# ecmwf/anemoi-core

Measured on AMD Instinct MI355X. Metric: forward nodes*channels/sec on O96 GraphTransformer, higher is better.
Workload: dtype bf16; 1 GPU; AnemoiModelEncProcDec forward, O96 data grid (40320 nodes, 84 vars x 2 steps) -> icosphere res 5 hidden mesh (10242 nodes, 81840 edges), GraphTransformer processor 16 layers x 512 ch x 16 heads, enc 62912 / dec 120960 edges, batch 1; parallelism=single GPU, hip_graph=True, graph_equals_eager=True, graph_segments=1

## Files before the change

### anemoi_core_amd/_lib.py

```python
from __future__ import annotations

import ctypes as C
import os
import threading

ABI_VERSION = 18
LIB_PATH = os.path.join(os.path.dirname(os.path.abspath(__file__)), "lib", "libanemoi_hip.so")

F32, BF16, F16 = 0, 1, 2
ACT_NONE, ACT_GELU = 0, 1
E_INVALID, E_UNSUPPORTED, E_LAUNCH = -1, -2, -3

_p, _i64, _i32, _f = C.c_void_p, C.c_int64, C.c_int32, C.c_float



class LinearPlan(C.Structure):
    _fields_ = [(name, _i32) for name in ("kernel", "tile_m", "tile_n", "pingpong", "stage_k", "mi", "wr", "kg", "stages", "epi", "main_rows",
                                          "tail_rows", "ln_tail_begin")]


SIGNATURES = {
    "anemoi_hip_abi_version": ([], C.c_int),
    "anemoi_hip_last_error": ([], C.c_char_p),
    "anemoi_gt_attention_fwd": ([_p, _i64, _p, _i64, _p, _i64, _p, _i64, _p, _p, _p, _i64, _p, _i64, _p, _i32, _i32, _i32, _i32, C.c_int, _p], C.c_int),
    "anemoi_gt_attention_bwd": ([_p, _i64, _p, _i64, _p, _i64, _p, _i64, _p, _i64, _p, _p, _i64, _p, _p, _p, _p, _p,
                                 _p, _i64, _p, _i64, _p, _i64, _p, _i64, _p, _p, _i32, _i32, _i32, _i32, _i32, C.c_int, _p], C.c_int),
    "anemoi_gt_attention_dropout_fwd": ([_p, _i64, _p, _i64, _p, _i64, _p, _i64, _p, _p, _p, _i64, _p, _i64, _p, _i32, _i32, _i32, _i32, _f, C.c_uint64,
                                         C.c_int, _p], C.c_int),
    "anemoi_gt_attention_dropout_bwd": ([_p, _i64, _p, _i64, _p, _i64, _p, _i64, _p, _i64, _p, _p, _i64, _p, _p, _p, _p, _p,
                                         _p, _i64, _p, _i64, _p, _i64, _p, _i64, _p, _p, _i32, _i32, _i32, _i32, _i32, _f, C.c_uint64, C.c_int, _p], C.c_int),
    "anemoi_attention_dropout_mask": ([_p, _i32, _i32, _f, C.c_uint64, _p], C.c_int),
    "anemoi_gt_attention_fused_edge_fwd": ([_p, _i64, _p, _i64, _p, _i64, _p, _i32, _p, _p, _p, _p, _p, _i64, _p, _i64, _p, _i32, _i32, _i32, _i32, C.c_int, _p], C.c_int),
    "anemoi_pack_edge_weights": ([_p, _p, _p, _i32, _i32, _i32, C.c_int, _p], C.c_int),
    "anemoi_pack_edge_features": ([_p, _i64, _p, _i32, _i32, _i32, C.c_int, _p], C.c_int),
    "anemoi_reduce_workspace_bytes": ([_i32], _i64),
    "anemoi_layernorm_bwd": ([_p, _i64, _p, _p, _i64, _p, _i64, _p, _p, _p, _i32, _i32, _f, C.c_int, _p], C.c_int),
    "anemoi_colsum": ([_p, _i64, _p, _p, _i32, _i32, C.c_int, _p], C.c_int),
    "anemoi_gelu_fwd": ([_p, _i64, _p, _i64, _i32, _i32, C.c_int, _p], C.c_int),
# ... 7 lines not shown
    "anemoi_assemble_output_norm": ([_p, _i64, C.c_int, _p, _i64, _p, _p, _p, _p, _i64, _i32, _i32, C.c_int, _p], C.c_int),
    "anemoi_affine_columns": ([_p, _i64, _p, _i64, _p, _p, _i32, _i32, _i32, C.c_int, _p], C.c_int),
    "anemoi_bound_columns": ([_p, _i64, _i32, _i32, _p, _p, _i32, C.c_int, _p], C.c_int),
    "anemoi_layernorm_fwd": ([_p, _i64, _p, _p, _p, _i64, _p, _i64, _i32, _i32, _f, C.c_int, _p], C.c_int),
    "anemoi_gt_attention_fused_edge_bwd_partial_floats": ([_i32, _i32, _i32], _i64),
    "anemoi_gt_attention_fused_edge_bwd": ([_p, _i64, _p, _i64, _p, _i64, _p, _i32, _p, _p, _i64, _p, _p, _i64, _p, _p, _p, _p, _p,
                                            _p, _i64, _p, _i64, _p, _i64, _p, _p, _p, _p, _p, _p, _p, _p, _i64, _p, _i64,
                                            _i32, _i32, _i32, _i32, _i32, C.c_int, _p], C.c_int),
    "anemoi_linear_wgrad_workspace_bytes": ([_i32, _i32, _i32], _i64),
    "anemoi_linear_wgrad": ([_p, _i64, _p, _i64, _p, _i64, _p, _p, _i32, _i32, _i32, C.c_int, _p], C.c_int),
    "anemoi_linear_splitk_f32": ([_p, _i64, _p, _i64, _p, _i64, _i32, _i32, _i32, _i32, C.c_int, _p], C.c_int),
    "anemoi_linear_stats_fwd": ([_p, _i64, _i32, _p, _i64, _p, _p, _i64, _p, _i64, _p, _i32, _i32, C.c_int, _p], C.c_int),
    "anemoi_linear_lnfold_fwd": ([_p, _i64, _i32, _p, _i64, _p, _p, _p, _i32, _f, C.c_int, _p, _i64, _i32, _i32, C.c_int, _p], C.c_int),
    "anemoi_linear_plan": ([_i32, _i32, _i32, _i32, _i32, _i32, C.c_int, C.POINTER(LinearPlan)], C.c_int),
    "anemoi_linear_fwd": ([_p, _i64, _i32, _p, _i64, _i32, _p, _i64, _p, _p, _i64, _p, _p, _i64, _p, _p, _i64, _p, _i64, _i32, _i32, C.c_int, C.c_int, _p], C.c_int),
    "anemoi_linear_fwd_pre": ([_p, _i64, _i32, _p, _i64, _i32, _p, _i64, _p, _p, _i64, _p, _p, _i64, _p, _p, _i64, _p, _i64, _p, _i64, _i32, _i32,
                               C.c_int, C.c_int, _p], C.c_int),
    "anemoi_edge_ln_residual_segment_sum_fwd": ([_p, _i64, _p, _i64, _p, _p, _f, _p, _p, _i64, _p, _i64, _i32, _i32, C.c_int, _p], C.c_int),
    "anemoi_segment_sum_rows": ([_p, _i64, _p, _p, _p, _i64, _i32, _i32, C.c_int, _p], C.c_int),
    "anemoi_gather_add_rows": ([_p, _i64, _p, _i64, _p, _p, _i64, _i32, _i32, C.c_int, _p], C.c_int),
    "anemoi_transpose_pad": ([_p, _i64, _p, _i64, _i32, _i32, _i32, C.c_int, _p], C.c_int),
    "anemoi_glu_fwd": ([_p, _i64, _p, _i64, _i32, _i32, _i32, C.c_int, _p], C.c_int),
    "anemoi_glu_bwd": ([_p, _i64, _p, _i64, _p, _i64, _i32, _i32, _i32, C.c_int, _p], C.c_int),
    "anemoi_gather_rows": ([_p, _i64, _p, _p, _i64, _i32, _i32, C.c_int, _p], C.c_int),
    "anemoi_peer_alloc": ([C.POINTER(_p), _i64, _i32], C.c_int),
    "anemoi_peer_free": ([_p], C.c_int),
    "anemoi_peer_export": ([_p, _p], C.c_int),
    "anemoi_peer_open": ([_p, C.POINTER(_p)], C.c_int),
    "anemoi_peer_close": ([_p], C.c_int),
    "anemoi_gt_chain_rows_per_tile": ([_i32], C.c_int),
    "anemoi_gt_chain2_fwd": ([_p, C.c_int, _p], C.c_int),
    "anemoi_gt_rowchain_fwd": ([_p, C.c_int, _p], C.c_int),
    "anemoi_gt_rowchain_panels_fwd": ([_p, C.c_int32, C.c_int32, C.c_int, _p], C.c_int),
    "anemoi_gt_chain2_side_fwd": ([_p, _p, C.c_int32, C.c_int32, C.c_int32, C.c_int, _p], C.c_int),
    "anemoi_gt_cluster_chain_fwd": ([_p, C.c_int, _p], C.c_int),
    "anemoi_gt_cluster_chain_workspace_bytes": ([], _i64),
    "anemoi_gnn_edge_chain_fwd": ([_p, _i64, _p, _i64, _p, _p, _i64, _p, _p, _p, _p, _p, _p, _p, _p, _p, _f, _p, _i64, _i32, _i32, C.c_int, _p], C.c_int),
    "anemoi_gnn_mlp_chain_fwd": ([_p, _i64, _i32, _p, _p, _p, _p, _p, _p, _p, _p, _f, _p, _i64, _p, _i64, _i32, _i32, C.c_int, _p], C.c_int),
    "anemoi_gnn_node_chain_segsum_fwd": ([_p, _i64, _p, _i64, _p, _p, _p, _p, _p, _p, _p, _p, _p, _f, _p, _i64, _p, _p, _i32, _p, _i64, _i32, _i32,
                                          C.c_int, _p], C.c_int),
    "anemoi_gnn_node_chain_fwd": ([_p, _i64, _p, _i64, _p, _p, _p, _p, _p, _p, _p, _p, _f, _p, _i64, _p, _p, _i32, _p, _i64, _i32, _i32, C.c_int, _p], C.c_int),
    "anemoi_peer_exchange_rows": ([_p, _i64, _p, _p, _i32, _i32, _i32, _p, _p, _i64, _p], C.c_int),
    "anemoi_window_attention_fwd": ([_p, _i64, _p, _i64, _p, _i64, _p, _i64, _p, _i32, _i32, _i32, _i32, _i32, _f, _f, _p, C.c_int, _p], C.c_int),
    "anemoi_sparse_project_fwd": ([_p, _i64, _i64, _i32, _i64, _i32, _i32, _p, _p, _p, _p, _p, _p, _p, _i64, _i64, _i32, _i32, _i32, C.c_int, C.c_int, _p], C.c_int),
}


EXPERIMENT_SIGNATURES = {
    "anemoi_gt_chain_fwd": ([_p, C.c_int, _p], C.c_int),
    "anemoi_gnn_edge_chain_timeline": ([_p, _i64, _p, _i64, _p, _p, _i64, _p, _p, _p, _p, _p, _p, _p, _p, _p, _f, _p, _i64, _i32, _p, _p], C.c_int),
}


class HipLibraryError(RuntimeError):
    pass


_lock = threading.Lock()
_lib = None


def load(path: str | None = None):
    global _lib
    if _lib is not None:
        return _lib
    with _lock:
# ... 40 lines not shown
```

### anemoi_core_amd/build.py

```python
from __future__ import annotations

import os
import shutil
import subprocess
import sys
from concurrent.futures import ThreadPoolExecutor

PKG = os.path.dirname(os.path.abspath(__file__))
REPO = os.path.dirname(PKG)
CSRC = os.path.join(PKG, "csrc")
LIBDIR = os.path.join(PKG, "lib")
LIBPATH = os.path.join(LIBDIR, "libanemoi_hip.so")
EXT_PATH = os.path.join(LIBDIR, "libanemoi_torch.so")
INCLUDE = os.path.join(REPO, "include")

SOURCES = ["lib.cpp", "gt_attention.hip", "gt_attention_bwd.hip", "rowwise.hip", "rowwise_bwd.hip", "linear.hip", "wgrad.hip", "peer.hip", "gt_chain2.hip", "gt_chain2_side.hip", "gt_rowchain.hip", "gt_cluster_chain.hip", "gnn_chain.hip", "window_attention.hip", "sparse_project.hip"]
EXPERIMENT_SOURCES = ["experiments/gt_chain.hip", "experiments/gnn_chain2.hip"]
EXP_LIBPATH = os.path.join(LIBDIR, "libanemoi_hip_exp.so")
ARCH = "gfx950"


def _hipcc() -> str:
    for cand in (os.environ.get("HIPCC"), shutil.which("hipcc"), "/opt/rocm/bin/hipcc"):
        if cand and os.path.exists(cand):
            return cand
    raise RuntimeError("hipcc not found (need ROCm >= 7.0)")


def _newer(target: str, deps: list[str]) -> bool:
    if not os.path.exists(target):
        return False
    t = os.path.getmtime(target)
    return all(os.path.getmtime(d) <= t for d in deps)


def _deps(path: str, dirs: list[str], seen: set | None = None) -> list[str]:
    import re

    seen = set() if seen is None else seen
    if path in seen:
        return []
    seen.add(path)
    out = [path]
    for inc in re.findall(r'^\s*#include\s+"([^"]+)"', open(path).read(), flags=re.M):
        for d in [os.path.dirname(path), *dirs]:
            cand = os.path.join(d, inc)
            if os.path.exists(cand):
                out += _deps(cand, dirs, seen)
                break
# ... 65 lines not shown
```

### anemoi_core_amd/layers/mapper.py

```python
from __future__ import annotations

import os
from typing import Optional

import torch
from torch import Tensor, nn

from .. import ops
from ..distributed import primitives as comm
from ..distributed.partition import (
    build_graph_partition_from_shard_info,
    ensure_edges_are_dst_sorted,
    local_bipartite_graph,
    shard_edges_1hop,
)
from ..distributed.shapes import BipartiteGraphShardInfo, comm_rank, comm_size, get_shard_sizes, model_is_distributed
from .block import GraphConvMapperBlock, GraphTransformerMapperBlock
from .handoff import Carrier, SideJob, inference_in, plain_layer_norm
from .kernels import PaddedLinear
from .mlp import MLP
from .utils import compute_mlp_hidden_dim, load_layer_kernels
from ..utils.tensors import version


_ROW_CHAIN = os.environ.get("ANEMOI_ROW_CHAIN", "1") != "0"
_ROW_CHAIN_MIN_ROWS = int(os.environ.get("ANEMOI_ROW_CHAIN_MIN_ROWS", "4096"))
_TAIL_PROJ = os.environ.get("ANEMOI_TAIL_PROJ", "1") != "0"
_ENC_DST_CACHE = os.environ.get("ANEMOI_ENC_DST_CACHE", "1") != "0"
_ROW_CHAIN_GEMM_BAND = tuple(int(v) for v in os.environ.get("ANEMOI_ROW_CHAIN_GEMM_BAND", "16384:262144").split(":"))


class _LocalGraphCache:

    def __init__(self, keep: int = 4):
        self.entries: dict = {}
        self.keep = keep

    def get(self, key, build):
        hit = self.entries.get(key)
        if hit is None:
            hit = build()
            if len(self.entries) >= self.keep:
                self.entries.pop(next(iter(self.entries)))
            self.entries[key] = hit
        return hit


class BaseMapper(nn.Module):
    def __init__(self, *, in_channels_src: int, in_channels_dst: int, hidden_dim: int, out_channels_dst: Optional[int] = None,
                 cpu_offload: bool = False, gradient_checkpointing: bool = True, layer_kernels=None, **kwargs) -> None:
        super().__init__()
        self.in_channels_src = in_channels_src
        self.in_channels_dst = in_channels_dst
        self.hidden_dim = hidden_dim
        self.out_channels_dst = out_channels_dst
        self.gradient_checkpointing = gradient_checkpointing
        self.layer_factory = load_layer_kernels(layer_kernels)
        if cpu_offload:
            raise NotImplementedError("cpu_offload is a training memory feature; not needed with 288 GB of HBM")
        self._local = _LocalGraphCache()
        self._heads_cache = None

# ... 52 lines not shown

    def _tail_projection(self):
        return None

    def _row_chain_ok(self, x: Tensor, lin, ln, projs: list, band: bool = True) -> bool:
        return (_ROW_CHAIN and x.is_cuda and x.dim() == 2 and x.dtype != torch.float32 and x.shape[0] >= _ROW_CHAIN_MIN_ROWS
                and not (band and _ROW_CHAIN_GEMM_BAND[0] < x.shape[0] < _ROW_CHAIN_GEMM_BAND[1])
                and self.hidden_dim == ops.CHAIN_CHANNELS and plain_layer_norm(ln) and lin.in_features <= x.shape[1] and lin.bias is not None
                and ops.gt_row_chain_supported(x, sum(p.out_features for p in projs)) and all(p.in_features == ops.CHAIN_CHANNELS for p in projs)
                and inference_in(x, lin, ln, *projs))

    def _row_chain_operands(self, x: Tensor, lin, side: str, band: bool = True):
        blk = self.proc
        ln = blk.layer_norm_attention_src if side == "src" else blk.layer_norm_attention_dest
        projs = [blk.lin_key, blk.lin_value] if side == "src" else [blk.lin_query, blk.lin_self]
        if not self._row_chain_ok(x, lin, ln, projs, band):
            return None
        params = [lin.weight, lin.bias, ln.weight, ln.bias] + [q for m in projs for q in (m.weight, m.bias)]
        K = x.shape[1]

        def build():
            w = lin.weight if lin.in_features == K else torch.nn.functional.pad(lin.weight, (0, K - lin.in_features))
            wq = torch.cat([m.weight for m in projs], dim=0)
            bq = torch.cat([m.bias if m.bias is not None else m.weight.new_zeros(m.out_features) for m in projs])
            wqg, dq = ops.fold_layer_norm(wq, bq, ln.weight, ln.bias)
            return ops.pack_embedding_frag(w), ops.pack_weight_frag(wqg), torch.cat([lin.bias.float(), dq]).to(x.dtype).contiguous(), wq.shape[0]

        return (*blk._fused.derived(f"rowchain:{side}:{K}", params, build), ln.eps)

    def _row_chain(self, x: Tensor, lin, side: str, want_x: bool):
        operands = self._row_chain_operands(x, lin, side)
        return None if operands is None else ops.gt_row_chain(x, *operands, want_x_out=want_x)

    def _static_row_chain(self, x: Tensor, lin):
        blk = self.proc
        ln, projs = blk.layer_norm_attention_dest, [blk.lin_query, blk.lin_self]
        params = [x, lin.weight, lin.bias, ln.weight, ln.bias] + [q for m in projs for q in (m.weight, m.bias)]
        return blk._fused.derived(f"rowchain-static:dst:{x.shape[1]}", params, lambda: (self._row_chain(x, lin, "dst", True), x))[0]

    def destination_side_job(self, x_dst: Tensor, panels_per_rider: int) -> Optional[SideJob]:
        operands = self._row_chain_operands(x_dst, self.emb_nodes_dst, "dst", band=False)
        if operands is None:
            return None
        we, wqg, vec, q_out, eps = operands
        n, dt, dev = x_dst.shape[0], x_dst.dtype, x_dst.device
        return SideJob(x=x_dst, we=we, wqg=wqg, vec=vec, q_out_features=q_out, ln_eps=eps, y=torch.empty((n, self.hidden_dim), dtype=dt, device=dev),
                       q=torch.empty((n, q_out), dtype=dt, device=dev), panels_per_rider=panels_per_rider)

    def _embed(self, padded: PaddedLinear, x: Tensor, lin, side: str, carrier: Optional[Carrier]) -> Tensor:
        ln = self.proc.layer_norm_attention_src if side == "src" else self.proc.layer_norm_attention_dest
        if carrier is not None and side == "dst" and carrier.side_job is not None and carrier.side_job.x is x:
            job, carrier.side_job = carrier.side_job, None
            job.finish()
            return carrier.put(job.y, proj=job.q)
        if carrier is not None:
            if _ENC_DST_CACHE and side == "dst" and carrier.static_dst is x and not torch.is_grad_enabled():
                r = self._static_row_chain(x, lin)
            else:
                r = self._row_chain(x, lin, side, want_x=side == "dst" or self.proc.update_src_nodes)
            if r is not None:
                y, proj = r
                return carrier.put(y if y is not None else x.new_empty((x.shape[0], 0)), proj=proj)
            if self.proc._ln_fold_ok(ln, x):
                y, stats = padded.with_row_stats(x, lin)
                return y if stats is None else carrier.put(y, stats=stats)
        return padded(x, lin)

    @comm.scoped_forward
    def forward(self, x, batch_size: int, shard_info: BipartiteGraphShardInfo, edge_attr: Tensor, edge_index: Tensor,
                model_comm_group=None, keep_x_dst_sharded: bool = False, edges_are_dst_sorted: bool = True, cond=None, **kwargs):
        if self.shard_strategy == "heads" and model_is_distributed(model_comm_group):
            return self._forward_heads(x, batch_size, shard_info, edge_attr, edge_index, model_comm_group, keep_x_dst_sharded,
                                       edges_are_dst_sorted, cond=cond, **kwargs)
        x_src, x_dst = x
        edge_attr, edge_index = ensure_edges_are_dst_sorted(
            edge_attr, edge_index, edges_are_sharded=shard_info.edges_are_sharded(), model_comm_group=model_comm_group,
            edges_are_dst_sorted=edges_are_dst_sorted)
        g = self._local_graph(x, shard_info, edge_attr, edge_index, model_comm_group)
        d0, d1 = g["dst_range"]
        sharded = model_is_distributed(model_comm_group)
        if sharded and not shard_info.dst_is_sharded():
            x_dst = x_dst[d0:d1]
        if sharded and shard_info.src_is_sharded():
            x_src_c, g["plans"]["src"] = comm.exchange_rows(x_src, g["src_ids"], shard_info.src_nodes, model_comm_group,
                                                            gather_fn=ops.gather_rows, plan=g["plans"].get("src"))
        elif g["all_connected"]:
            x_src_c = x_src
        else:
# ... 204 lines not shown
```

### anemoi_core_amd/ops.py

```python
from __future__ import annotations

from dataclasses import dataclass
from typing import NamedTuple, Optional

import os

import torch
from torch import Tensor

from . import _ext, _lib

_DT = {torch.float32: _lib.F32, torch.bfloat16: _lib.BF16, torch.float16: _lib.F16}


def _dt(t: Tensor) -> int:
    try:
        return _DT[t.dtype]
    except KeyError:
        raise ValueError(f"unsupported dtype {t.dtype}; supported: float32, bfloat16, float16") from None


try:
    _raw_stream = torch._C._cuda_getCurrentRawStream
except AttributeError:
# ... 1069 lines not shown
    q_out = torch.empty((N, q_out_features), dtype=dt, device=x.device)
    a = _row_chain_args(x, we, wqg, vec, q_out_features, ln_eps, x_out, q_out, rows_per_tile)
    _lib.check(_lib.load().anemoi_gt_rowchain_fwd(_lib.C.byref(a), _dt(x), _stream()), "gt_rowchain_fwd")
    return x_out, q_out


def gt_row_chain_panels(x: Tensor, we: Tensor, wqg: Tensor, vec: Tensor, q_out_features: int, ln_eps: float, y: Optional[Tensor], q: Tensor,
                        first_panel: int, panels: int) -> None:
    a = _row_chain_args(x, we, wqg, vec, q_out_features, ln_eps, y, q, 0)
    _lib.check(_lib.load().anemoi_gt_rowchain_panels_fwd(_lib.C.byref(a), int(first_panel), int(panels), _dt(x), _stream()), "gt_rowchain_panels_fwd")


def _row_chain_args(x: Tensor, we: Tensor, wqg: Tensor, vec: Tensor, q_out_features: int, ln_eps: float, x_out: Optional[Tensor], q_out: Tensor,
                    rows_per_tile: int) -> _RowChainArgs:
    _dev(x, we, wqg, vec, x_out, q_out)
    N, K = x.shape
    dt, D = x.dtype, CHAIN_CHANNELS
    if not gt_row_chain_supported(x, q_out_features):
        raise NotImplementedError(f"gt_row_chain: x {tuple(x.shape)} {dt} / q_out={q_out_features} (16-bit rows of <= {D} columns, a multiple of 8; q_out a multiple of {D})")
    kp = (K + 127) // 128 * 128
    for name, w, numel in (("we", we, D * kp), ("wqg", wqg, q_out_features * D)):
        if w.dim() != 1 or w.numel() != numel or w.dtype != dt or not w.is_contiguous():
            raise ValueError(f"gt_row_chain: {name} must be the contiguous fragment-major image ({numel} x {dt})")
    if vec.dim() != 1 or vec.numel() != D + q_out_features or vec.dtype != dt or not vec.is_contiguous():
        raise ValueError(f"gt_row_chain: vec must be contiguous [{D + q_out_features}] {dt} = cat[be, dq]")
    for name, t, cols in (("x_out", x_out, D), ("q_out", q_out, q_out_features)):
        if t is not None and (tuple(t.shape) != (N, cols) or t.dtype != dt or not t.is_contiguous()):
            raise ValueError(f"gt_row_chain: {name} must be contiguous [{N}, {cols}] {dt}")
    xp, ldx = _rows(x, "x", dt)
    return _RowChainArgs(xp, ldx, K, we.data_ptr(), wqg.data_ptr(), q_out_features, vec.data_ptr(), float(ln_eps),
                         0 if x_out is None else x_out.data_ptr(), D, q_out.data_ptr(), q_out_features, N, D, int(rows_per_tile))


def gnn_edge_chain(e: Tensor, g1: Tensor, idx1: Tensor, g2: Tensor, idx2: Tensor, w0: Tensor, b0: Tensor, w1: Tensor, b1: Tensor, w2: Tensor,
                   b2: Tensor, ln_w: Tensor, ln_b: Optional[Tensor], eps: float) -> Tensor:
    _dev(e, g1, idx1, g2, idx2, w0, b0, w1, b1, w2, b2, ln_w, ln_b)
    M, D = e.shape
    dt = e.dtype
    if D != CHAIN_CHANNELS or dt not in (torch.bfloat16, torch.float16):
        raise NotImplementedError(f"gnn_edge_chain: {D} channels / {dt} (built for {CHAIN_CHANNELS} channels, 16-bit dtypes)")
    for name, w in (("w0", w0), ("w1", w1), ("w2", w2)):
        if w.dim() != 1 or w.numel() != D * D or w.dtype != dt or not w.is_contiguous():
            raise ValueError(f"gnn_edge_chain: {name} must be the fragment-major image of a [{D}, {D}] weight (pack_weight_frag)")
    for name, ix in (("idx1", idx1), ("idx2", idx2)):
        if ix.dtype != torch.int32 or ix.dim() != 1 or ix.shape[0] != M or not ix.is_contiguous():
            raise ValueError(f"gnn_edge_chain: {name} must be contiguous int32 [{M}]")
    if g1.shape[1] != D or g2.shape[1] != D:
        raise ValueError("gnn_edge_chain: the gathered tables must have 512 columns")
    out = torch.empty((M, D), dtype=dt, device=e.device)
    (ep, lde), (p1, ld1), (p2, ld2) = _rows(e, "e", dt), _rows(g1, "g1", dt), _rows(g2, "g2", dt)
    _lib.check(_lib.load().anemoi_gnn_edge_chain_fwd(ep, lde, p1, ld1, idx1.data_ptr(), p2, ld2, idx2.data_ptr(), w0.data_ptr(), _vec(b0, "b0", D, dt),
                                                     w1.data_ptr(), _vec(b1, "b1", D, dt), w2.data_ptr(), _vec(b2, "b2", D, dt), _vec(ln_w, "ln_w", D, dt),
                                                     _vec(ln_b, "ln_b", D, dt), float(eps), out.data_ptr(), D, M, D, _dt(e), _stream()), "gnn_edge_chain_fwd")
    return out


def gnn_mlp_chain(x: Tensor, w0: Tensor, b0: Tensor, w1: Tensor, b1: Tensor, w2: Tensor, b2: Tensor, ln_w: Tensor, ln_b: Optional[Tensor],
                  eps: float, residual: Optional[Tensor] = None) -> Tensor:
    _dev(x, w0, b0, w1, b1, w2, b2, ln_w, ln_b, residual)
    N, K = x.shape
    D, dt = CHAIN_CHANNELS, x.dtype
    if dt not in (torch.bfloat16, torch.float16) or K % 128 or not 128 <= K <= D:
        raise NotImplementedError(f"gnn_mlp_chain: width {K} / {dt} (built for 16-bit rows of 128, 256, 384 or 512 columns)")
    for name, w, numel in (("w0", w0, D * K), ("w1", w1, D * D), ("w2", w2, D * D)):
        if w.dim() != 1 or w.numel() != numel or w.dtype != dt or not w.is_contiguous():
            raise ValueError(f"gnn_mlp_chain: {name} must be a contiguous fragment-major image of {numel} elements (pack_weight_frag)")
# ... 231 lines not shown
```

### include/anemoi_hip.h

```cpp
#ifndef ANEMOI_HIP_H
#define ANEMOI_HIP_H

#include <stdint.h>

#ifdef __cplusplus
extern "C" {
#endif

#define ANEMOI_HIP_ABI_VERSION 18

typedef enum { ANEMOI_F32 = 0, ANEMOI_BF16 = 1, ANEMOI_F16 = 2 } anemoi_dtype_t;
typedef enum { ANEMOI_ACT_NONE = 0, ANEMOI_ACT_GELU = 1 } anemoi_act_t;

#define ANEMOI_OK 0
#define ANEMOI_E_INVALID (-1)
#define ANEMOI_E_UNSUPPORTED (-2)
#define ANEMOI_E_LAUNCH (-3)

int anemoi_hip_abi_version(void);
const char* anemoi_hip_last_error(void);

int anemoi_gt_attention_fwd(const void* q, int64_t ldq, const void* k, int64_t ldk, const void* v, int64_t ldv,
                            const void* e, int64_t lde, const int32_t* row, const int32_t* colptr,
                            const void* addend, int64_t ldadd, void* out, int64_t ldo, float* lse,
                            int32_t n_dst, int32_t n_src, int32_t H, int32_t C, anemoi_dtype_t dtype, void* stream);

int anemoi_gt_attention_bwd(const void* q, int64_t ldq, const void* k, int64_t ldk, const void* v, int64_t ldv,
                            const void* e, int64_t lde, const void* out, int64_t ldo, const float* lse,
                            const void* d_out, int64_t lddo, const int32_t* row, const int32_t* colptr,
                            const int32_t* rowptr, const int32_t* edge_ids, const int32_t* edge_dst,
                            void* dq, int64_t lddq, void* dk, int64_t lddk, void* dv, int64_t lddv, void* de, int64_t ldde,
                            float* p_ws, float* ds_ws, int32_t n_dst, int32_t n_src, int32_t n_edges, int32_t H, int32_t C,
                            anemoi_dtype_t dtype, void* stream);

int anemoi_gt_attention_dropout_fwd(const void* q, int64_t ldq, const void* k, int64_t ldk, const void* v, int64_t ldv,
                                    const void* e, int64_t lde, const int32_t* row, const int32_t* colptr,
                                    const void* addend, int64_t ldadd, void* out, int64_t ldo, float* lse,
                                    int32_t n_dst, int32_t n_src, int32_t H, int32_t C, float drop_p, uint64_t drop_seed,
                                    anemoi_dtype_t dtype, void* stream);
int anemoi_gt_attention_dropout_bwd(const void* q, int64_t ldq, const void* k, int64_t ldk, const void* v, int64_t ldv,
                                    const void* e, int64_t lde, const void* out, int64_t ldo, const float* lse,
                                    const void* d_out, int64_t lddo, const int32_t* row, const int32_t* colptr,
// ... 141 lines not shown
                              int64_t timeout_ticks, void* stream);

typedef struct anemoi_gt_chain2_args {
  const void* attn;   int64_t ld_attn;
  const void* x_res;  int64_t ld_x;
  const void* wp;
  const void* w1;     int32_t hidden;
  const void* w2;
  const void* wq;     int32_t q_out_features;
  const void* vec;
  float ln1_eps;      float lnq_eps;
  const void* extra;  int64_t ld_extra;
  void* x_out;        int64_t ld_out;
  void* q_out;        int64_t ld_q;
  int32_t n_rows;     int32_t channels;   int32_t rows_per_tile;
  void* timeline;
} anemoi_gt_chain2_args_t;
int anemoi_gt_chain2_fwd(const anemoi_gt_chain2_args_t* args, anemoi_dtype_t dtype, void* stream);
int anemoi_gt_chain_rows_per_tile(int32_t n_rows);

typedef struct anemoi_gt_rowchain_args {
  const void* x;      int64_t ld_x;       int32_t in_features;
  const void* we;
  const void* wq;     int32_t q_out_features;
  const void* vec;
  float ln_eps;
  void* x_out;        int64_t ld_out;
  void* q_out;        int64_t ld_q;
  int32_t n_rows;     int32_t channels;   int32_t rows_per_tile;
} anemoi_gt_rowchain_args_t;
int anemoi_gt_rowchain_fwd(const anemoi_gt_rowchain_args_t* args, anemoi_dtype_t dtype, void* stream);
int anemoi_gt_rowchain_panels_fwd(const anemoi_gt_rowchain_args_t* args, int32_t first_panel, int32_t panels, anemoi_dtype_t dtype, void* stream);

int anemoi_gt_chain2_side_fwd(const anemoi_gt_chain2_args_t* args, const anemoi_gt_rowchain_args_t* side, int32_t side_first_panel,
                              int32_t side_panels, int32_t side_blocks, anemoi_dtype_t dtype, void* stream);

typedef struct anemoi_gt_cluster_chain_args {
  const void* attn;   int64_t ld_attn;
  const void* x_res;  int64_t ld_x;
  const void* wp;
  const void* w1;     int32_t hidden;
  const void* w2;
  const void* wq;     int32_t q_out_features;
  const void* vec;
  float ln1_eps;      float lnq_eps;
  const void* extra;  int64_t ld_extra;
  void* x_out;        int64_t ld_out;
  void* q_out;        int64_t ld_q;
  void* ln_out;       int64_t ld_ln;
  void* q_out2;       int64_t ld_q2;      int32_t q_split;
  void* workspace;    int64_t workspace_bytes;
  int32_t n_rows;     int32_t channels;
} anemoi_gt_cluster_chain_args_t;
int anemoi_gt_cluster_chain_fwd(const anemoi_gt_cluster_chain_args_t* args, anemoi_dtype_t dtype, void* stream);
int64_t anemoi_gt_cluster_chain_workspace_bytes(void);

int anemoi_gnn_edge_chain_fwd(const void* e, int64_t ld_e, const void* g1, int64_t ld_g1, const int32_t* idx1, const void* g2, int64_t ld_g2,
                              const int32_t* idx2, const void* w0, const void* b0, const void* w1, const void* b1, const void* w2, const void* b2,
                              const void* ln_w, const void* ln_b, float eps, void* e_new, int64_t ld_o, int32_t n_rows, int32_t channels,
                              anemoi_dtype_t dtype, void* stream);
int anemoi_gnn_mlp_chain_fwd(const void* x, int64_t ld_x, int32_t in_features, const void* w0, const void* b0, const void* w1, const void* b1,
                             const void* w2, const void* b2, const void* ln_w, const void* ln_b, float eps, const void* res, int64_t ld_res,
                             void* out, int64_t ld_o, int32_t n_rows, int32_t channels, anemoi_dtype_t dtype, void* stream);

int anemoi_gnn_node_chain_fwd(const void* x, int64_t ld_x, const void* agg, int64_t ld_a, const void* wa, const void* ba, const void* wb,
                              const void* bb, const void* wc, const void* bc, const void* ln_w, const void* ln_b, float eps, void* x_out,
// ... 24 lines not shown
```

Before: 9.206 billion nodes*channels/s.

## Fold encoder source embedding, LayerNorm and K/V projection into one kernel

Adds a kernel for the encoder source side that computes the embedding GEMM only for LayerNorm row statistics. It then applies K/V projection weights folded with the embedding weights (Wc = Wp·diag(gamma)·We) straight from the raw input, giving the LN output algebraically as rstd·(Wc x + u) − mu·rstd·s + d. This avoids writing the 512-channel embedded source rows and running a separate LN+projection chain when source nodes are not updated, so one GEMM over 512-wide hidden rows is replaced by a narrow-K GEMM. The cost is precision: the composed weight is rounded to 16-bit and the embedding is recomputed, so results differ slightly from the unfused path.

```diff
diff --git a/anemoi_core_amd/_lib.py b/anemoi_core_amd/_lib.py
--- a/anemoi_core_amd/_lib.py
+++ b/anemoi_core_amd/_lib.py
@@ -4,7 +4,7 @@
 import os
 import threading
 
-ABI_VERSION = 18
+ABI_VERSION = 19
 LIB_PATH = os.path.join(os.path.dirname(os.path.abspath(__file__)), "lib", "libanemoi_hip.so")
 
 F32, BF16, F16 = 0, 1, 2
@@ -78,6 +78,7 @@
     "anemoi_gt_chain2_fwd": ([_p, C.c_int, _p], C.c_int),
     "anemoi_gt_rowchain_fwd": ([_p, C.c_int, _p], C.c_int),
     "anemoi_gt_rowchain_panels_fwd": ([_p, C.c_int32, C.c_int32, C.c_int, _p], C.c_int),
+    "anemoi_gt_embed_fold_fwd": ([_p, C.c_int, _p], C.c_int),
     "anemoi_gt_chain2_side_fwd": ([_p, _p, C.c_int32, C.c_int32, C.c_int32, C.c_int, _p], C.c_int),
     "anemoi_gt_cluster_chain_fwd": ([_p, C.c_int, _p], C.c_int),
     "anemoi_gt_cluster_chain_workspace_bytes": ([], _i64),
diff --git a/anemoi_core_amd/build.py b/anemoi_core_amd/build.py
--- a/anemoi_core_amd/build.py
+++ b/anemoi_core_amd/build.py
@@ -14,7 +14,7 @@
 EXT_PATH = os.path.join(LIBDIR, "libanemoi_torch.so")
 INCLUDE = os.path.join(REPO, "include")
 
-SOURCES = ["lib.cpp", "gt_attention.hip", "gt_attention_bwd.hip", "rowwise.hip", "rowwise_bwd.hip", "linear.hip", "wgrad.hip", "peer.hip", "gt_chain2.hip", "gt_chain2_side.hip", "gt_rowchain.hip", "gt_cluster_chain.hip", "gnn_chain.hip", "window_attention.hip", "sparse_project.hip"]
+SOURCES = ["lib.cpp", "gt_attention.hip", "gt_attention_bwd.hip", "rowwise.hip", "rowwise_bwd.hip", "linear.hip", "wgrad.hip", "peer.hip", "gt_chain2.hip", "gt_chain2_side.hip", "gt_rowchain.hip", "gt_embed_fold.hip", "gt_cluster_chain.hip", "gnn_chain.hip", "window_attention.hip", "sparse_project.hip"]
 EXPERIMENT_SOURCES = ["experiments/gt_chain.hip", "experiments/gnn_chain2.hip"]
 EXP_LIBPATH = os.path.join(LIBDIR, "libanemoi_hip_exp.so")
 ARCH = "gfx950"
diff --git a/anemoi_core_amd/csrc/gt_embed_fold.hip b/anemoi_core_amd/csrc/gt_embed_fold.hip
--- /dev/null
+++ b/anemoi_core_amd/csrc/gt_embed_fold.hip
@@ -0,0 +1,214 @@
+#include "chain_core.h"
+
+namespace anemoi {
+
+constexpr int kEfRows = 80, kEfBands = 5, kEfWaves = 4, kEfThreads = 64 * kEfWaves;
+constexpr int kEfRowBytes = 512;
+constexpr int kEfRedOff = kEfRows * kEfRowBytes;
+constexpr int kEfStripOff = kEfRedOff + kEfRows * 4 * 2 * 4;
+constexpr int kEfStripBytes = 16 * 256;
+constexpr int kEfVecOff = kEfStripOff + kEfWaves * kEfStripBytes;
+constexpr int kEfMaxQ = 2048;
+constexpr int kEfVecMax = kCh + 3 * kEfMaxQ;
+constexpr int ef_smem(int qc) { return kEfVecOff + (kCh + 3 * kCh * qc) * 4; }
+constexpr int kEfXIt = kEfRows * 32 / kEfThreads, kEfVecIt = (kEfVecMax / 4 + kEfThreads - 1) / kEfThreads;
+static_assert(ef_smem(kEfMaxQ / kCh) <= 160 * 1024, "LDS budget");
+
+struct EmbedFoldArgs {
+  const void* x;   int64_t ld_x;  int k_in;
+  const char* we;  const char* wc;
+  int nks, qc;
+  const float* vec;
+  float eps;
+  void* qout;      int64_t ld_q;
+  int n_rows;
+};
+
+template <typename T>
+__device__ __forceinline__ void embed_fold_gemm(const unsigned char* arow, int x, int ks, frag8 (&ring)[8], const char* cur, int64_t cs, const char* nxt,
+                                                int64_t ns, uint32_t loff, f32x4 (&acc)[kEfBands][8], int nks) {
+  frag8 fa[kEfBands];
+#pragma unroll
+  for (int mi = 0; mi < kEfBands; ++mi) fa[mi] = *reinterpret_cast<const frag8*>(arow + mi * 16 * kEfRowBytes + ((ks ^ x) << 4));
+#pragma unroll 1
+  for (int st = 0; st < nks; ++st) {
+    const bool last = st == nks - 1;
+    const gptr_t g0 = uniform_ptr(last ? nxt : cur + (st + 1) * 4096), g1 = uniform_ptr(last ? nxt + ns : cur + cs + (st + 1) * 4096);
+    const int aoff = ((((last ? st : st + 1) * 4 + ks) ^ x) << 4);
+#pragma unroll
+    for (int ni = 0; ni < 8; ++ni) {
+#pragma unroll
+      for (int mi = 0; mi < kEfBands; ++mi) {
+        acc[mi][ni] = cmfma<T>(ring[ni], fa[mi], acc[mi][ni]);
+        if (ni == 7) fa[mi] = *reinterpret_cast<const frag8*>(arow + mi * 16 * kEfRowBytes + aoff);
+      }
+      ring[ni] = *reinterpret_cast<gfrag_t>((ni < 4 ? g0 : g1) + loff + (ni & 3) * 1024);
+      __builtin_amdgcn_sched_barrier(0);
+    }
+  }
+}
+
+template <typename T>
+__global__ __launch_bounds__(kEfThreads, 2) void gt_embed_fold_kernel(EmbedFoldArgs a) {
+  extern __shared__ __attribute__((aligned(16))) unsigned char smem[];
+  float* const red = reinterpret_cast<float*>(smem + kEfRedOff);
+  float* const vec = reinterpret_cast<float*>(smem + kEfVecOff);
+  const int tid = threadIdx.x, lane = tid & 63;
+  const int c = __builtin_amdgcn_readfirstlane(tid >> 6);
+  const uint32_t loff = lane * 16;
+  const int x = lane & 15, g = lane >> 4;
+  const int r0 = (int)blockIdx.x * kEfRows, nr = min(kEfRows, a.n_rows - r0);
+  const int nks = a.nks, qc = a.qc;
+  const int64_t slab = (int64_t)nks * 4096;
+  const char* const we = a.we + (int64_t)(2 * c) * slab;
+  auto wcp = [&](int p) { return a.wc + (int64_t)(8 * p + 2 * c) * slab; };
+  frag8 ring[8];
+  {
+    const int spr = nks * 4, n = kEfRows * spr, kin16 = a.k_in >> 3;
+    const int nv = (kCh + 3 * kCh * qc) / 4;
+    u32x4 v[kEfXIt], vv[kEfVecIt];
+#pragma unroll
+    for (int k = 0; k < kEfXIt; ++k) {
+      const int i = tid + kEfThreads * k;
+      if (k * kEfThreads < n) {
+        const int row = min(i / spr, kEfRows - 1), slot = i % spr;
+        const bool live = row < nr && slot < kin16 && i < n;
+        const unsigned char* p = reinterpret_cast<const unsigned char*>(a.x) + ((int64_t)(r0 + min(row, nr - 1)) * a.ld_x + min(slot, kin16 - 1) * 8) * 2;
+        const u32x4 t = stream_load(reinterpret_cast<const u32x4*>(p));
+        v[k] = live ? t : u32x4{0u, 0u, 0u, 0u};
+      }
+    }
+#pragma unroll
+    for (int k = 0; k < kEfVecIt; ++k)
+      if (k * kEfThreads < nv) vv[k] = reinterpret_cast<const u32x4*>(a.vec)[min(tid + kEfThreads * k, nv - 1)];
+    {
+      const gptr_t g0 = uniform_ptr(we), g1 = uniform_ptr(we + slab);
+#pragma unroll
+      for (int ni = 0; ni < 8; ++ni) ring[ni] = *reinterpret_cast<gfrag_t>((ni < 4 ? g0 : g1) + loff + (ni & 3) * 1024);
+    }
+#pragma unroll
+    for (int k = 0; k < kEfXIt; ++k) {
+      const int i = tid + kEfThreads * k;
+      if (i < n) {
+        const int row = i / spr, slot = i % spr;
+        *reinterpret_cast<u32x4*>(smem + row * kEfRowBytes + ((slot ^ (row & 15)) << 4)) = v[k];
+      }
+    }
+#pragma unroll
+    for (int k = 0; k < kEfVecIt; ++k)
+      if (tid + kEfThreads * k < nv) reinterpret_cast<u32x4*>(vec)[tid + kEfThreads * k] = vv[k];
+    lds_barrier();
+  }
+  const unsigned char* const arow = smem + x * kEfRowBytes;
+  f32x4 acc[kEfBands][8];
+#pragma unroll
+  for (int ni = 0; ni < 8; ++ni) {
+    const f32x4 b = *reinterpret_cast<const f32x4*>(vec + c * 128 + ni * 16 + g * 4);
+#pragma unroll
+    for (int mi = 0; mi < kEfBands; ++mi) acc[mi][ni] = b;
+  }
+  embed_fold_gemm<T>(arow, x, g, ring, we, slab, wcp(0), slab, loff, acc, nks);
+#pragma unroll
+  for (int mi = 0; mi < kEfBands; ++mi) {
+#pragma unroll
+    for (int ni = 0; ni < 8; ++ni) {
+      float o[4] = {acc[mi][ni][0], acc[mi][ni][1], acc[mi][ni][2], acc[mi][ni][3]};
+      unpack4<T>(pack4<T>(o), o);
+      acc[mi][ni] = f32x4{o[0], o[1], o[2], o[3]};
+    }
+    const float2 p = row_partial<8>(acc[mi]);
+    if (g == 0) *reinterpret_cast<float2*>(red + ((mi * 16 + x) * 4 + c) * 2) = p;
+  }
+  lds_barrier();
+  float ra[kEfBands], rb[kEfBands];
+#pragma unroll
+  for (int mi = 0; mi < kEfBands; ++mi) {
+    float mu, rstd;
+    merge_partials<4>(red, mi * 16 + x, a.eps, mu, rstd);
+    ra[mi] = rstd;
+    rb[mi] = -mu * rstd;
+  }
+  unsigned char* const strip = smem + kEfStripOff + c * kEfStripBytes;
+  const float* const vu = vec + kCh;
+  const float* const vs = vu + kCh * qc;
+  const float* const vd = vs + kCh * qc;
+  T* const out = static_cast<T*>(a.qout);
+#pragma unroll 1
+  for (int p = 0; p < qc; ++p) {
+    const int col0 = p * kCh + c * 128;
+#pragma unroll
+    for (int ni = 0; ni < 8; ++ni) {
+      const f32x4 u = *reinterpret_cast<const f32x4*>(vu + col0 + ni * 16 + g * 4);
+#pragma unroll
+      for (int mi = 0; mi < kEfBands; ++mi) acc[mi][ni] = u;
+    }
+    const char* const cur = wcp(p);
+    embed_fold_gemm<T>(arow, x, g, ring, cur, slab, p + 1 < qc ? wcp(p + 1) : cur, slab, loff, acc, nks);
+    int le = lane;
+    asm volatile("" : "+v"(le));
+    const int xe = le & 15, ge = le >> 4;
+    T* const orow = out + (int64_t)(r0 + ge) * a.ld_q + col0 + xe * 8;
+#pragma unroll
+    for (int mi = 0; mi < kEfBands; ++mi) {
+#pragma unroll
+      for (int ni = 0; ni < 8; ++ni) {
+        const f32x4 s4 = *reinterpret_cast<const f32x4*>(vs + col0 + ni * 16 + ge * 4);
+        const f32x4 d4 = *reinterpret_cast<const f32x4*>(vd + col0 + ni * 16 + ge * 4);
+        float o[4];
+#pragma unroll
+        for (int r = 0; r < 4; ++r) o[r] = fmaf(ra[mi], acc[mi][ni][r], fmaf(rb[mi], s4[r], d4[r]));
+        *reinterpret_cast<u32x2*>(strip + xe * 256 + (((ni * 2 + (ge >> 1)) ^ xe) << 4) + (ge & 1) * 8) = pack4<T>(o);
+      }
+      asm volatile("s_waitcnt lgkmcnt(0)" ::: "memory");
+#pragma unroll
+      for (int it = 0; it < 4; ++it) {
+        const int sr = it * 4 + ge, row = mi * 16 + sr;
+        const u32x4 t = *reinterpret_cast<const u32x4*>(strip + sr * 256 + ((xe ^ sr) << 4));
+        if (row < nr) stream_store(t, reinterpret_cast<u32x4*>(orow + (int64_t)(mi * 16 + it * 4) * a.ld_q));
+      }
+      asm volatile("s_waitcnt lgkmcnt(0)" ::: "memory");
+    }
+  }
+}
+
+template <typename T>
+static int launch_embed_fold(const EmbedFoldArgs& a, hipStream_t st) {
+  static PerDeviceOnce once;
+  once.run([&] {
+    (void)hipFuncSetAttribute(reinterpret_cast<const void*>(&gt_embed_fold_kernel<T>), hipFuncAttributeMaxDynamicSharedMemorySize, ef_smem(kEfMaxQ / kCh));
+  });
+  const int grid = (a.n_rows + kEfRows - 1) / kEfRows;
+  hipLaunchKernelGGL((gt_embed_fold_kernel<T>), dim3(grid), dim3(kEfThreads), ef_smem(a.qc), st, a);
+  return check_launch("gt_embed_fold_kernel");
+}
+
+}
+
+using namespace anemoi;
+
+extern "C" int anemoi_gt_embed_fold_fwd(const anemoi_gt_embed_fold_args_t* p, anemoi_dtype_t dtype, void* stream) {
+  const char* who = "gt_embed_fold_fwd";
+  ANEMOI_REQUIRE(p != nullptr, "%s: null argument block", who);
+  ANEMOI_REQUIRE(p->n_rows >= 0 && p->in_features > 0 && p->q_out_features > 0, "%s: n_rows=%d in_features=%d q_out_features=%d", who, p->n_rows,
+                 p->in_features, p->q_out_features);
+  if ((dtype != ANEMOI_BF16 && dtype != ANEMOI_F16) || p->channels != kCh || p->in_features > 256 || p->in_features % 8 != 0 ||
+      p->q_out_features % kCh != 0 || p->q_out_features > kEfMaxQ) {
+    set_error("%s: not eligible (16-bit dtypes, 512 channels, in_features a multiple of 8 up to 256, q_out_features a multiple of 512 up to %d)", who, kEfMaxQ);
+    return ANEMOI_E_UNSUPPORTED;
+  }
+  if (p->n_rows == 0) return ANEMOI_OK;
+  ANEMOI_REQUIRE(p->x && p->we && p->wc && p->vec && p->q_out, "%s: null operand", who);
+  const auto al16 = [](const void* q) { return (reinterpret_cast<uintptr_t>(q) & 15) == 0; };
+  ANEMOI_REQUIRE(al16(p->x) && al16(p->we) && al16(p->wc) && al16(p->vec) && al16(p->q_out), "%s: operands must be 16-byte aligned", who);
+  ANEMOI_REQUIRE(p->ld_x >= p->in_features && p->ld_x % 8 == 0 && p->ld_q >= p->q_out_features && p->ld_q % 8 == 0,
+                 "%s: leading dimensions too small or not multiples of 8 elements", who);
+  EmbedFoldArgs a;
+  a.x = p->x; a.ld_x = p->ld_x; a.k_in = p->in_features;
+  a.we = static_cast<const char*>(p->we); a.wc = static_cast<const char*>(p->wc);
+  a.nks = 2 * ((p->in_features + 63) / 64); a.qc = p->q_out_features / kCh;
+  a.vec = p->vec; a.eps = p->ln_eps;
+  a.qout = p->q_out; a.ld_q = p->ld_q;
+  a.n_rows = p->n_rows;
+  hipStream_t st = as_stream(stream);
+  return dtype == ANEMOI_BF16 ? launch_embed_fold<bf16_t>(a, st) : launch_embed_fold<f16_t>(a, st);
+}
diff --git a/anemoi_core_amd/layers/mapper.py b/anemoi_core_amd/layers/mapper.py
--- a/anemoi_core_amd/layers/mapper.py
+++ b/anemoi_core_amd/layers/mapper.py
@@ -28,6 +28,7 @@
 _TAIL_PROJ = os.environ.get("ANEMOI_TAIL_PROJ", "1") != "0"
 _ENC_DST_CACHE = os.environ.get("ANEMOI_ENC_DST_CACHE", "1") != "0"
 _ROW_CHAIN_GEMM_BAND = tuple(int(v) for v in os.environ.get("ANEMOI_ROW_CHAIN_GEMM_BAND", "16384:262144").split(":"))
+_EMBED_FOLD = os.environ.get("ANEMOI_EMBED_FOLD", "1") != "0"
 
 
 class _LocalGraphCache:
@@ -146,6 +147,25 @@
         operands = self._row_chain_operands(x, lin, side)
         return None if operands is None else ops.gt_row_chain(x, *operands, want_x_out=want_x)
 
+    def _embed_fold(self, x: Tensor, lin) -> Optional[Tensor]:
+        blk = self.proc
+        ln, projs = blk.layer_norm_attention_src, [blk.lin_key, blk.lin_value]
+        q_out = sum(m.out_features for m in projs)
+        if not (_EMBED_FOLD and _ROW_CHAIN_GEMM_BAND[0] < x.shape[0] < _ROW_CHAIN_GEMM_BAND[1] and self.hidden_dim == ops.CHAIN_CHANNELS
+                and plain_layer_norm(ln) and lin.in_features <= x.shape[1] and all(m.in_features == ops.CHAIN_CHANNELS for m in projs)
+                and ops.gt_embed_fold_supported(x, q_out) and inference_in(x, lin, ln, *projs)):
+            return None
+        params = [lin.weight, lin.bias, ln.weight, ln.bias] + [q for m in projs for q in (m.weight, m.bias)]
+        K = x.shape[1]
+
+        def build():
+            w = lin.weight if lin.in_features == K else torch.nn.functional.pad(lin.weight, (0, K - lin.in_features))
+            wq = torch.cat([m.weight for m in projs], dim=0)
+            bq = torch.cat([m.bias if m.bias is not None else m.weight.new_zeros(m.out_features) for m in projs])
+            return ops.compose_embedding_projection(w, lin.bias, wq, bq, ln.weight, ln.bias)
+
+        return ops.gt_embed_fold(x, *blk._fused.derived(f"embed-fold:src:{K}", params, build), q_out, ln.eps)
+
     def _static_row_chain(self, x: Tensor, lin):
         blk = self.proc
         ln, projs = blk.layer_norm_attention_dest, [blk.lin_query, blk.lin_self]
@@ -168,6 +188,10 @@
             job.finish()
             return carrier.put(job.y, proj=job.q)
         if carrier is not None:
+            if side == "src" and not self.proc.update_src_nodes:
+                kv = self._embed_fold(x, lin)
+                if kv is not None:
+                    return carrier.put(x.new_empty((x.shape[0], 0)), proj=kv)
             if _ENC_DST_CACHE and side == "dst" and carrier.static_dst is x and not torch.is_grad_enabled():
                 r = self._static_row_chain(x, lin)
             else:
diff --git a/anemoi_core_amd/ops.py b/anemoi_core_amd/ops.py
--- a/anemoi_core_amd/ops.py
+++ b/anemoi_core_amd/ops.py
@@ -1125,6 +1125,57 @@
                          0 if x_out is None else x_out.data_ptr(), D, q_out.data_ptr(), q_out_features, N, D, int(rows_per_tile))
 
 
+class _EmbedFoldArgs(_lib.C.Structure):
+    _p, _i64, _i32, _f = _lib.C.c_void_p, _lib.C.c_int64, _lib.C.c_int32, _lib.C.c_float
+    _fields_ = [("x", _p), ("ld_x", _i64), ("in_features", _i32), ("we", _p), ("wc", _p), ("q_out_features", _i32), ("vec", _p), ("ln_eps", _f),
+                ("q_out", _p), ("ld_q", _i64), ("n_rows", _i32), ("channels", _i32)]
+
+
+EMBED_FOLD_MAX_IN = 256
+
+
+def compose_embedding_projection(w_emb: Tensor, b_emb: Optional[Tensor], w_proj: Tensor, b_proj: Optional[Tensor], gamma: Tensor,
+                                 beta: Optional[Tensor]) -> tuple[Tensor, Tensor, Tensor]:
+    dt = w_emb.dtype
+    we, wp = w_emb.detach().float(), w_proj.detach().float()
+    be = we.new_zeros(we.shape[0]) if b_emb is None else b_emb.detach().float()
+    bp = wp.new_zeros(wp.shape[0]) if b_proj is None else b_proj.detach().float()
+    wg = wp * gamma.detach().float()
+    d = bp if beta is None else wp @ beta.detach().float() + bp
+    pad = (-we.shape[1]) % 64
+    wc = torch.nn.functional.pad((wg @ we).to(dt), (0, pad))
+    we16 = torch.nn.functional.pad(w_emb.detach(), (0, pad))
+    return pack_weight_frag(we16), pack_weight_frag(wc), torch.cat([be, wg @ be, wg.sum(dim=1), d]).contiguous()
+
+
+def gt_embed_fold_supported(x: Tensor, q_out: int) -> bool:
+    return (x.is_cuda and x.dim() == 2 and x.dtype in (torch.bfloat16, torch.float16) and 0 < x.shape[1] <= EMBED_FOLD_MAX_IN
+            and x.shape[1] % 8 == 0 and x.stride(1) == 1 and x.stride(0) % 8 == 0 and q_out > 0 and q_out % CHAIN_CHANNELS == 0
+            and q_out <= 4 * CHAIN_CHANNELS)
+
+
+def gt_embed_fold(x: Tensor, we: Tensor, wc: Tensor, vec: Tensor, q_out_features: int, ln_eps: float) -> Optional[Tensor]:
+    _dev(x, we, wc, vec)
+    if not gt_embed_fold_supported(x, q_out_features):
+        return None
+    N, K = x.shape
+    dt, D = x.dtype, CHAIN_CHANNELS
+    kp = (K + 63) // 64 * 64
+    for name, w, numel in (("we", we, D * kp), ("wc", wc, q_out_features * kp)):
+        if w.dim() != 1 or w.numel() != numel or w.dtype != dt or not w.is_contiguous():
+            raise ValueError(f"gt_embed_fold: {name} must be the contiguous fragment-major image ({numel} x {dt}) made by compose_embedding_projection")
+    if vec.dim() != 1 or vec.numel() != D + 3 * q_out_features or vec.dtype != torch.float32 or not vec.is_contiguous():
+        raise ValueError(f"gt_embed_fold: vec must be contiguous fp32 [{D + 3 * q_out_features}] = cat[be, u, s, d]")
+    q_out = torch.empty((N, q_out_features), dtype=dt, device=x.device)
+    xp, ldx = _rows(x, "x", dt)
+    a = _EmbedFoldArgs(xp, ldx, K, we.data_ptr(), wc.data_ptr(), q_out_features, vec.data_ptr(), float(ln_eps), q_out.data_ptr(), q_out_features, N, D)
+    rc = _lib.load().anemoi_gt_embed_fold_fwd(_lib.C.byref(a), _dt(x), _stream())
+    if rc == _lib.E_UNSUPPORTED:
+        return None
+    _lib.check(rc, "gt_embed_fold_fwd")
+    return q_out
+
+
 def gnn_edge_chain(e: Tensor, g1: Tensor, idx1: Tensor, g2: Tensor, idx2: Tensor, w0: Tensor, b0: Tensor, w1: Tensor, b1: Tensor, w2: Tensor,
                    b2: Tensor, ln_w: Tensor, ln_b: Optional[Tensor], eps: float) -> Tensor:
     _dev(e, g1, idx1, g2, idx2, w0, b0, w1, b1, w2, b2, ln_w, ln_b)
diff --git a/include/anemoi_hip.h b/include/anemoi_hip.h
--- a/include/anemoi_hip.h
+++ b/include/anemoi_hip.h
@@ -7,7 +7,7 @@
 extern "C" {
 #endif
 
-#define ANEMOI_HIP_ABI_VERSION 18
+#define ANEMOI_HIP_ABI_VERSION 19
 
 typedef enum { ANEMOI_F32 = 0, ANEMOI_BF16 = 1, ANEMOI_F16 = 2 } anemoi_dtype_t;
 typedef enum { ANEMOI_ACT_NONE = 0, ANEMOI_ACT_GELU = 1 } anemoi_act_t;
@@ -215,6 +215,16 @@
 int anemoi_gt_rowchain_fwd(const anemoi_gt_rowchain_args_t* args, anemoi_dtype_t dtype, void* stream);
 int anemoi_gt_rowchain_panels_fwd(const anemoi_gt_rowchain_args_t* args, int32_t first_panel, int32_t panels, anemoi_dtype_t dtype, void* stream);
 
+typedef struct anemoi_gt_embed_fold_args {
+  const void* x;      int64_t ld_x;       int32_t in_features;
+  const void* we;
+  const void* wc;     int32_t q_out_features;
+  const float* vec;   float ln_eps;
+  void* q_out;        int64_t ld_q;
+  int32_t n_rows;     int32_t channels;
+} anemoi_gt_embed_fold_args_t;
+int anemoi_gt_embed_fold_fwd(const anemoi_gt_embed_fold_args_t* args, anemoi_dtype_t dtype, void* stream);
+
 int anemoi_gt_chain2_side_fwd(const anemoi_gt_chain2_args_t* args, const anemoi_gt_rowchain_args_t* side, int32_t side_first_panel,
                               int32_t side_panels, int32_t side_blocks, anemoi_dtype_t dtype, void* stream);
 
```

Measured after the change: 9.344 billion nodes*channels/s, median of 6. +1.5%, better.
